# vitskvara/VBMatrixFactorization.jl

Measured on NVIDIA B200. Metric: VB iterations/s at 20000x200000x64 (dense vbmf, Float64), higher is better.
Workload: dtype f64

## Files before the change

vbmatrixfactorization.jl_b200/csrc/capi.cu:

```cuda
#include "../../include/vbmf_b200.h"
#include "common.cuh"
#include "gemm.cuh"
#include "kernels.cuh"

#include <atomic>
#include <type_traits>
#include <cstdarg>
#include <cstdlib>
#include <cstring>
#include <dlfcn.h>
#include <unistd.h>
#include <string>
#include <vector>
#include <algorithm>
#include <thread>

namespace vb {

static thread_local char g_err[1024] = "";
void set_error(const char* fmt, ...) {
    va_list ap;
    va_start(ap, fmt);
    vsnprintf(g_err, sizeof(g_err), fmt, ap);
    va_end(ap);
// ... 275 lines not shown
        if (comm_in != nullptr) c->comm = comm_in;
        else {
            if (nccl_id128 == nullptr) { set_error("world > 1 needs the NCCL unique id of rank 0"); delete c; return -1; }
            if (load_nccl()) { delete c; return -1; }
            NcclUniqueId id;
            memcpy(&id, nccl_id128, 128);
            int r = g_nccl.CommInitRank(&c->comm, c->world, id, rank);
            if (r != 0) { set_error("ncclCommInitRank failed: %s", g_nccl.GetErrorString ? g_nccl.GetErrorString(r) : "?"); delete c; return -1; }
        }
    }
    if (cudaMalloc(&c->d_tr, 64) != cudaSuccess) { set_error("cudaMalloc failed"); delete c; return -1; }
    *out = c;
    return 0;
}
extern "C" int vbmf_b200_ctx_create(int device, int rank, int world, const void* nccl_id128, void* cuda_stream,
                                    vbmf_b200_ctx** out) {
    return ctx_create_impl(device, rank, world, nccl_id128, nullptr, cuda_stream, out);
}
namespace vb {
int ctx_create_with_comm(int device, int rank, int world, void* comm, vbmf_b200_ctx** out) {
    return ctx_create_impl(device, rank, world, nullptr, comm, nullptr, out);
}
int nccl_comm_init_all(void** comms, int ndev, const int* devs) {
    if (load_nccl()) return -1;
    if (!g_nccl.CommInitAll) { set_error("the NCCL library has no ncclCommInitAll"); return -1; }
    VB_NCCL_OK(g_nccl.CommInitAll(comms, ndev, devs));
    return 0;
}
}

static void ctx_free_Z(vbmf_b200_ctx* c) {
    if (c->Z) cudaFree(c->Z);
    if (c->Zexp) cudaFree(c->Zexp);
    c->Z = nullptr; c->Zexp = nullptr; c->Z_bytes = 0;
    c->z_ready = false; c->z_failed = false;
}

static void ctx_free_Y(vbmf_b200_ctx* c) {
    ctx_free_Z(c);
    if (c->copy_st) cudaStreamSynchronize(c->copy_st);
    if (c->stat_st) cudaStreamSynchronize(c->stat_st);
    c->chunks_pending = 0; c->tr_pending = false;
    if (c->Y) cudaFree(c->Y);
    if (c->rowY2) cudaFree(c->rowY2);
    if (c->stats_part) cudaFree(c->stats_part);
    c->Y = nullptr; c->rowY2 = nullptr; c->stats_part = nullptr; c->have_Y = false;
    c->Y_cap = 0; c->L_cap = 0;
}

extern "C" int vbmf_b200_ctx_destroy(vbmf_b200_ctx* c) {
    if (!c) return 0;
    cudaSetDevice(c->device);
    cudaStreamSynchronize(c->st);
    ctx_free_Y(c);
    if (c->d_tr) cudaFree(c->d_tr);
    px_release(c);
    if (c->px.wait_ns) cudaFree(c->px.wait_ns);
    if (c->batch_dev) cudaFree(c->batch_dev);
    if (c->batch_host) cudaFreeHost(c->batch_host);
    for (auto e : c->ev_k1) cudaEventDestroy(e);
    for (auto e : c->ev_k2) cudaEventDestroy(e);
    for (auto e : c->ev_ar) cudaEventDestroy(e);
    for (auto& e : c->ev_seg) cudaEventDestroy(e.second);
    for (auto e : c->ev_chunk) cudaEventDestroy(e);
    if (c->ev_stats) cudaEventDestroy(c->ev_stats);
    if (c->copy_st) { cudaStreamSynchronize(c->copy_st); cudaStreamDestroy(c->copy_st); }
    if (c->stat_st) { cudaStreamSynchronize(c->stat_st); cudaStreamDestroy(c->stat_st); }
    if (c->comm) g_nccl.CommDestroy(c->comm);
    if (c->own_stream) cudaStreamDestroy(c->st);
    delete c;
    return 0;
}

extern "C" int vbmf_b200_ctx_sync(vbmf_b200_ctx* c) {
    VB_CUDA_OK(cudaSetDevice(c->device));
    if (c->copy_st) VB_CUDA_OK(cudaStreamSynchronize(c->copy_st));
    if (c->stat_st) VB_CUDA_OK(cudaStreamSynchronize(c->stat_st));
    VB_CUDA_OK(cudaStreamSynchronize(c->st));
    return 0;
}

static int ctx_alloc_Y(vbmf_b200_ctx* c, int64_t L, int64_t Mloc, int64_t Mglob, int64_t off) {
    if (L <= 0 || Mloc < 0 || Mglob < Mloc || off < 0 || off + Mloc > Mglob) { set_error("bad Y geometry L=%lld M_local=%lld M_global=%lld offset=%lld", (long long)L, (long long)Mloc, (long long)Mglob, (long long)off); return -1; }
    if (L > 0x7fffff00LL || Mglob > 0x7fffff00LL) { set_error("L and M must fit in 31 bits"); return -1; }
    VB_CUDA_OK(cudaSetDevice(c->device));
    VB_CUDA_OK(cudaStreamSynchronize(c->st));
    if (c->copy_st) VB_CUDA_OK(cudaStreamSynchronize(c->copy_st));
    if (c->stat_st) VB_CUDA_OK(cudaStreamSynchronize(c->stat_st));
    c->chunks_pending = 0; c->tr_pending = false;
    const int ld = (int)((L + 1) & ~1LL);
    const size_t bytes = std::max<size_t>((size_t)ld * (size_t)std::max<int64_t>(Mloc, 1) * 8, 16);
    const bool reuse = c->Y != nullptr && c->rowY2 != nullptr && c->stats_part != nullptr && bytes <= c->Y_cap &&
                       c->Y_cap <= 2 * bytes + (64u << 20) && L <= c->L_cap;
    if (!reuse) {
        ctx_free_Y(c);
        VB_CUDA_OK(cudaMalloc(&c->Y, bytes));
        c->Y_cap = bytes;
        VB_CUDA_OK(cudaMalloc(&c->rowY2, (size_t)L * 8));
        VB_CUDA_OK(cudaMalloc(&c->stats_part, (size_t)(MAX_PARTS / 2) * L * 8));
        c->L_cap = (int)L;
    }
    c->have_Y = false;
    c->z_ready = false; c->z_failed = false;
    c->L = (int)L; c->Mloc = (int)Mloc; c->Mglob = (int)Mglob; c->moff = (int)off;
    c->ldY = ld;
    if (c->ldY != L) VB_CUDA_OK(cudaMemsetAsync(c->Y, 0, bytes, c->st));
    return 0;
}

static int ctx_finish_Y(vbmf_b200_ctx* c) {
    if (c->Mloc > 0) {
        if (make_tmap_2d(&c->tmY1, c->Y, (uint64_t)c->L, (uint64_t)c->Mloc, (uint64_t)c->ldY * 8, 16, 128)) return -1;
        if (make_tmap_2d(&c->tmY2, c->Y, (uint64_t)c->L, (uint64_t)c->Mloc, (uint64_t)c->ldY * 8, 16, 16)) return -1;
    }
    Dev d;
    memset(&d, 0, sizeof(d));
    d.L = c->L; d.Mloc = c->Mloc; d.Y = c->Y; d.ldY = c->ldY; d.rowY2 = c->rowY2; d.part = c->stats_part;
    if (k_y_stats(c->st, d, c->d_tr)) return -1;
    if (c->world > 1) {
        if (ctx_allreduce(c, c->rowY2, (size_t)c->L)) return -1;
        if (k_total(c->st, c->rowY2, c->L, c->d_tr)) return -1;
    }
    VB_CUDA_OK(cudaMemcpyAsync(&c->trYTY, c->d_tr, 8, cudaMemcpyDeviceToHost, c->st));
    VB_CUDA_OK(cudaStreamSynchronize(c->st));
    c->have_Y = true;
    return 0;
}

static int ctx_wait_upload(vbmf_b200_ctx* c) {
    if (c->chunks_pending > 0) {
        VB_CUDA_OK(cudaStreamWaitEvent(c->st, c->ev_stats, 0));
        c->chunks_pending = 0;
    }
    return 0;
}
static int ctx_host_trYTY(vbmf_b200_ctx* c) {
    if (c->tr_pending) {
        VB_CUDA_OK(cudaEventSynchronize(c->ev_stats));
        VB_CUDA_OK(cudaMemcpy(&c->trYTY, c->d_tr, 8, cudaMemcpyDeviceToHost));
        c->tr_pending = false;
    }
    return 0;
}
static size_t align_up(size_t x, size_t a) { return (x + a - 1) / a * a; }

static bool ctx_int8_wanted(const vbmf_b200_ctx* c, int64_t H) {
    return !c->simt && !c->gemm_dmma && H >= 1 && H <= 64 && c->Y != nullptr && c->Mloc > 0;
}
static int ctx_slices(vbmf_b200_ctx* c, bool* ok) {
    *ok = false;
    if (c->z_failed || c->Y == nullptr || c->Mloc <= 0) return 0;
    if (c->z_ready) { *ok = true; return 0; }
    const int ldZ = i8_ld(c->L);
    const size_t bytes = (size_t)8 * c->Mloc * ldZ;
    if (c->Z == nullptr || c->Z_bytes != bytes || c->ldZ != ldZ) {
        ctx_free_Z(c);
        if (cudaMalloc(&c->Z, bytes) != cudaSuccess || cudaMalloc(&c->Zexp, ((size_t)c->L + c->Mloc) * 4) != cudaSuccess) {
            cudaGetLastError();
            ctx_free_Z(c);
            c->z_failed = true;
            return 0;
        }
        c->Z_bytes = bytes; c->ldZ = ldZ;
    }
    if (i8_build_Y(c->st, c->Y, c->ldY, c->L, c->Mloc, c->Z, ldZ, c->Zexp, c->Zexp + c->L)) return -1;
    const uint64_t s1 = (uint64_t)ldZ, s2 = (uint64_t)ldZ * c->Mloc;
    if (make_tmap_3d_i8(&c->tmZ1, c->Z, (uint64_t)c->L, (uint64_t)c->Mloc, 8, s1, s2, 32, 128, 8, false)) return -1;
    if (make_tmap_3d_i8(&c->tmZ2, c->Z, (uint64_t)c->L, (uint64_t)c->Mloc, 8, s1, s2, 128, 32, 8, true)) return -1;
    c->z_ready = true;
    *ok = true;
    return 0;
}
static void i8_plans(int L, int M, int H, int num_sms, int* S1, int* kbs1, int* S, int* kchunk) {
    plan_splitk_ytb(L, M, H, num_sms, S1, kbs1);
    *kbs1 = (*kbs1 + 1) & ~1;
    const int nkb = (L + 15) / 16;
    *S1 = std::max(1, (nkb + *kbs1 - 1) / *kbs1);
    plan_splitk(L, M, H, num_sms, S, kchunk);
    *kchunk = (*kchunk + 31) / 32 * 32;
    *S = std::max(1, (M + *kchunk - 1) / *kchunk);
}
struct I8Operands {
    char* mem = nullptr;
    uint8_t *Wb = nullptr, *Wa = nullptr;
    int *Gb = nullptr, *Ga = nullptr;
    int ldM = 0;
    CUtensorMap tmWb, tmWa;
    I8Operands() = default;
    I8Operands(const I8Operands&) = delete;
    I8Operands& operator=(const I8Operands&) = delete;
    ~I8Operands() { if (mem) cudaFree(mem); }
};
static int i8_operands_alloc(I8Operands* o, int L, int M, int H, int S, bool* ok) {
    *ok = false;
    const int Hp = i8_hpad(H), ldZ = i8_ld(L);
    o->ldM = i8_ld(std::max(M, 1));
    const size_t nb = align_up((size_t)8 * Hp * ldZ, 256), na = align_up((size_t)8 * Hp * o->ldM, 256);
    const size_t gb = align_up((size_t)Hp * 4, 256), ga = align_up((size_t)S * Hp * 4, 256);
    if (cudaMalloc(&o->mem, nb + na + gb + ga) != cudaSuccess) { cudaGetLastError(); o->mem = nullptr; return 0; }
    o->Wb = (uint8_t*)o->mem; o->Wa = o->Wb + nb; o->Gb = (int*)(o->Wa + na); o->Ga = (int*)((char*)o->Gb + gb);
    if (make_tmap_3d_i8(&o->tmWb, o->Wb, (uint64_t)L, (uint64_t)Hp, 8, (uint64_t)ldZ, (uint64_t)ldZ * Hp, 32, (uint32_t)Hp, 8, false)) return -1;
    if (M > 0 && make_tmap_3d_i8(&o->tmWa, o->Wa, (uint64_t)M, (uint64_t)Hp, 8, (uint64_t)o->ldM, (uint64_t)o->ldM * Hp, 32, (uint32_t)Hp, 8, false)) return -1;
    *ok = true;
    return 0;
}
static int i8_k1(vbmf_b200_ctx* c, I8Operands* o, const double* B, int ldB, int H, double* P, int S1, int kbs1, const Scalars* sc) {
    const int* F = c->Zexp;
    const int* E = c->Zexp + c->L;
    if (i8_slice_B(c->st, B, ldB, c->L, H, F, o->Wb, c->ldZ, o->Gb, sc)) return -1;
    return launch_gemm_i8(c->st, false, &c->tmZ1, &o->tmWb, P, c->Mloc, c->L, S1, kbs1 * 16, H, E, o->Gb, 0,
                          (size_t)c->Mloc * H, (size_t)H, 1, sc, c->num_sms);
}
static int i8_k2(vbmf_b200_ctx* c, I8Operands* o, const double* A, int H, double* Qpart, int ldQ, int S, int kchunk, const Scalars* sc) {
    const int* F = c->Zexp;
    const int* E = c->Zexp + c->L;
    if (i8_slice_A(c->st, A, c->Mloc, H, E, kchunk, S, o->Wa, o->ldM, o->Ga, sc)) return -1;
    return launch_gemm_i8(c->st, true, &c->tmZ2, &o->tmWa, Qpart, c->L, c->Mloc, S, kchunk, H, F, o->Ga, i8_hpad(H),
                          (size_t)H * ldQ, 1, (size_t)ldQ, sc, c->num_sms);
}

static int attach_Y_chunked(vbmf_b200_ctx* c, const double* Y, int64_t ldY, int64_t chunk_cols) {
    if (!c->copy_st) VB_CUDA_OK(cudaStreamCreateWithFlags(&c->copy_st, cudaStreamNonBlocking));
    if (!c->stat_st) VB_CUDA_OK(cudaStreamCreateWithFlags(&c->stat_st, cudaStreamNonBlocking));
    if (!c->ev_stats) VB_CUDA_OK(cudaEventCreateWithFlags(&c->ev_stats, cudaEventDisableTiming));
    c->chunk_c0.clear(); c->chunk_n.clear();
    for (int64_t c0 = 0; c0 < c->Mloc; c0 += chunk_cols) { c->chunk_c0.push_back((int)c0); c->chunk_n.push_back((int)std::min<int64_t>(chunk_cols, c->Mloc - c0)); }
    const size_t nch = c->chunk_c0.size();
    while (c->ev_chunk.size() < nch) { cudaEvent_t e; VB_CUDA_OK(cudaEventCreateWithFlags(&e, cudaEventDisableTiming)); c->ev_chunk.push_back(e); }
    cudaEvent_t e0;
    VB_CUDA_OK(cudaEventCreateWithFlags(&e0, cudaEventDisableTiming));
    VB_CUDA_OK(cudaEventRecord(e0, c->st));
    VB_CUDA_OK(cudaStreamWaitEvent(c->copy_st, e0, 0));
    VB_CUDA_OK(cudaStreamWaitEvent(c->stat_st, e0, 0));
    VB_CUDA_OK(cudaEventDestroy(e0));
    Dev d;
    memset(&d, 0, sizeof(d));
    d.L = c->L; d.Mloc = c->Mloc; d.Y = c->Y; d.ldY = c->ldY; d.rowY2 = c->rowY2; d.part = c->stats_part;
    for (size_t k = 0; k < nch; ++k) {
        const size_t c0 = (size_t)c->chunk_c0[k], n = (size_t)c->chunk_n[k];
        if (ldY == c->L && c->ldY == c->L)
            VB_CUDA_OK(cudaMemcpyAsync(c->Y + c0 * c->ldY, Y + c0 * (size_t)ldY, (size_t)c->L * n * 8, cudaMemcpyHostToDevice, c->copy_st));
        else
            VB_CUDA_OK(cudaMemcpy2DAsync(c->Y + c0 * c->ldY, (size_t)c->ldY * 8, Y + c0 * (size_t)ldY, (size_t)ldY * 8, (size_t)c->L * 8, n,
                                         cudaMemcpyHostToDevice, c->copy_st));
        VB_CUDA_OK(cudaEventRecord(c->ev_chunk[k], c->copy_st));
        VB_CUDA_OK(cudaStreamWaitEvent(c->stat_st, c->ev_chunk[k], 0));
        if (k_y_stats_chunk(c->stat_st, d, (int)c0, (int)n, k == 0 ? 1 : 0)) return -1;
    }
    if (c->world > 1) VB_NCCL_OK(g_nccl.AllReduce(c->rowY2, c->rowY2, (size_t)c->L, 8, 0, c->comm, c->stat_st));
    if (k_total(c->stat_st, c->rowY2, c->L, c->d_tr)) return -1;
    VB_CUDA_OK(cudaEventRecord(c->ev_stats, c->stat_st));
    if (make_tmap_2d(&c->tmY1, c->Y, (uint64_t)c->L, (uint64_t)c->Mloc, (uint64_t)c->ldY * 8, 16, 128)) return -1;
    if (make_tmap_2d(&c->tmY2, c->Y, (uint64_t)c->L, (uint64_t)c->Mloc, (uint64_t)c->ldY * 8, 16, 16)) return -1;
    c->chunks_pending = (int)nch;
    c->tr_pending = true;
    c->trYTY = nan("");
    c->have_Y = true;
    return 0;
}

extern "C" int vbmf_b200_attach_Y(vbmf_b200_ctx* c, const double* Y, int64_t L, int64_t M_local, int64_t ldY,
                                  int64_t M_global, int64_t col_offset) {
    if (!c || (!Y && M_local > 0)) { set_error("attach_Y: NULL argument"); return -1; }
    if (ldY < L) { set_error("attach_Y: ldY < L"); return -1; }
    if (ctx_alloc_Y(c, L, M_local, M_global, col_offset)) return -1;
    {
        const char* e = getenv("VBMF_B200_ATTACH_CHUNK_MB");
        const double chunk_mb = e ? atof(e) : 2048.0;
        const double col_bytes = (double)c->ldY * 8.0;
        int64_t chunk_cols = (int64_t)(chunk_mb * 1048576.0 / col_bytes) / 128 * 128;
        if (chunk_cols < 128) chunk_cols = 128;
        if (chunk_mb > 0 && M_local >= 2 * chunk_cols && !c->simt) return attach_Y_chunked(c, Y, ldY, chunk_cols);
    }
    if (M_local > 0) {
        if (ldY == L && c->ldY == L) {
            VB_CUDA_OK(cudaMemcpyAsync(c->Y, Y, (size_t)L * (size_t)M_local * 8, cudaMemcpyHostToDevice, c->st));
        } else {
            VB_CUDA_OK(cudaMemcpy2DAsync(c->Y, (size_t)c->ldY * 8, Y, (size_t)ldY * 8, (size_t)L * 8, (size_t)M_local,
                                         cudaMemcpyHostToDevice, c->st));
        }
    }
    return ctx_finish_Y(c);
}

extern "C" int vbmf_b200_set_shape(vbmf_b200_ctx* c, int64_t L, int64_t M_local, int64_t M_global, int64_t col_offset) {
    if (!c) { set_error("set_shape: NULL ctx"); return -1; }
    if (L <= 0 || M_local < 0 || M_global < M_local || col_offset < 0 || col_offset + M_local > M_global || L > 0x7fffff00LL || M_global > 0x7fffff00LL) {
        set_error("set_shape: bad geometry"); return -1;
    }
    VB_CUDA_OK(cudaSetDevice(c->device));
    VB_CUDA_OK(cudaStreamSynchronize(c->st));
    ctx_free_Y(c);
    c->L = (int)L; c->Mloc = (int)M_local; c->Mglob = (int)M_global; c->moff = (int)col_offset;
    c->ldY = (int)((L + 1) & ~1LL);
    c->trYTY = nan("");
    c->have_Y = true;
    return 0;
}

extern "C" int vbmf_b200_synth_Y(vbmf_b200_ctx* c, int64_t L, int64_t M_local, int64_t M_global, int64_t col_offset,
                                 int rank, double noise, uint64_t seed) {
    if (!c) { set_error("synth_Y: NULL ctx"); return -1; }
    if (ctx_alloc_Y(c, L, M_local, M_global, col_offset)) return -1;
    if (k_synth(c->st, c->Y, c->ldY, c->L, c->Mloc, c->moff, rank, noise, seed)) return -1;
    return ctx_finish_Y(c);
}

extern "C" int vbmf_b200_preprocess_Y(vbmf_b200_ctx* c, double lambda, int64_t* L_out, int64_t* used_rows) {
    if (!c || !c->have_Y || !c->Y) { set_error("preprocess_Y: no Y attached"); return -1; }
    VB_CUDA_OK(cudaSetDevice(c->device));
    if (ctx_wait_upload(c) || ctx_host_trYTY(c)) return -1;
    const int L = c->L, M = c->Mloc;
    cudaStream_t st = c->st;
    double *mu = nullptr, *den = nullptr, *rs = nullptr;
    VB_CUDA_OK(cudaMalloc(&mu, (size_t)L * 8));
    VB_CUDA_OK(cudaMalloc(&den, (size_t)L * 8));
    VB_CUDA_OK(cudaMalloc(&rs, (size_t)L * 8));
    int rc = 0;
    rc = k_row_pass(st, c->Y, c->ldY, L, M, 0, nullptr, nullptr, c->stats_part, mu);
    if (!rc) rc = ctx_allreduce(c, mu, (size_t)L);
    if (!rc) rc = k_finish_stats(st, mu, L, (double)c->Mglob, 0);
    if (!rc) rc = k_row_pass(st, c->Y, c->ldY, L, M, 1, mu, nullptr, c->stats_part, den);
    if (!rc) rc = ctx_allreduce(c, den, (size_t)L);
    if (!rc) rc = k_finish_stats(st, den, L, (double)c->Mglob, 1);
    if (!rc) rc = k_row_pass(st, c->Y, c->ldY, L, M, 2, mu, den, c->stats_part, rs);
    if (!rc) rc = ctx_allreduce(c, rs, (size_t)L);
    std::vector<double> hrs((size_t)L);
    if (!rc && cudaMemcpyAsync(hrs.data(), rs, (size_t)L * 8, cudaMemcpyDeviceToHost, st) != cudaSuccess) { set_error("preprocess_Y: copy failed"); rc = -1; }
    if (!rc && cudaStreamSynchronize(st) != cudaSuccess) { set_error("preprocess_Y: sync failed"); rc = -1; }
    cudaFree(mu); cudaFree(den); cudaFree(rs);
    if (rc) return rc;
    std::vector<int> rows;
    for (int l = 0; l < L; ++l) if (hrs[l] >= 1e-5) rows.push_back(l);
    const int Lnew = (int)rows.size();
    if (Lnew == 0) { set_error("preprocess_Y: every row is constant, nothing left"); return -1; }
    c->z_ready = false; c->z_failed = false;
    if (Lnew == L) {
        if (k_scale_all(st, c->Y, (size_t)c->ldY * (size_t)std::max(M, 1), lambda)) return -1;
    } else {
        const int ldn = (Lnew + 1) & ~1;
        double* Yn = nullptr;
        int* drows = nullptr;
        const size_t bytes = std::max<size_t>((size_t)ldn * (size_t)std::max(M, 1) * 8, 16);
        VB_CUDA_OK(cudaMalloc(&Yn, bytes));
        VB_CUDA_OK(cudaMalloc(&drows, (size_t)Lnew * 4));
        VB_CUDA_OK(cudaMemsetAsync(Yn, 0, bytes, st));
        VB_CUDA_OK(cudaMemcpyAsync(drows, rows.data(), (size_t)Lnew * 4, cudaMemcpyHostToDevice, st));
        if (k_compact_rows(st, c->Y, c->ldY, Yn, ldn, drows, Lnew, M, lambda)) return -1;
        VB_CUDA_OK(cudaStreamSynchronize(st));
        cudaFree(drows);
        cudaFree(c->Y);
        c->Y = Yn; c->Y_cap = bytes; c->L = Lnew; c->ldY = ldn;
    }
    if (L_out) *L_out = Lnew;
    if (used_rows) for (int k = 0; k < Lnew; ++k) used_rows[k] = rows[k] + 1;
// ... 1603 lines not shown
```

vbmatrixfactorization.jl_b200/csrc/gemm.cuh:

```cuda
#pragma once
#include "common.cuh"

namespace vb {

typedef CUresult (*PFN_encodeTiled)(CUtensorMap*, CUtensorMapDataType, cuuint32_t, void*, const cuuint64_t*,
                                    const cuuint64_t*, const cuuint32_t*, const cuuint32_t*, CUtensorMapInterleave,
                                    CUtensorMapSwizzle, CUtensorMapL2promotion, CUtensorMapFloatOOBfill);
PFN_encodeTiled tmap_encoder();

int make_tmap_2d(CUtensorMap* out, const void* base, uint64_t dim0, uint64_t dim1, uint64_t stride1_bytes,
                 uint32_t box0, uint32_t box1);

struct GemmGeometry {
    int bn;
    int ctas_per_sm;
    int stages;
};
GemmGeometry gemm_geometry(int H);
int gemm_init_device();

int launch_gemm_ytb(cudaStream_t st, const CUtensorMap* tmY, const CUtensorMap* tmB, double* P,
                    int M, int L, int H, int ldP, int S, int kb_per_split, size_t slab_stride, const Scalars* sc, int num_sms);
void plan_splitk_ytb(int L, int M, int H, int num_sms, int* S, int* kb_per_split);

int launch_gemm_ya(cudaStream_t st, const CUtensorMap* tmY, const CUtensorMap* tmA, double* Qpart,
                   int L, int M, int H, int ldQ, int kchunk, int S, const Scalars* sc, int num_sms);

int plan_streamk(int L, int M, int H, int num_sms, int* kq, int* nk, int* grid, int* smax);
int launch_gemm_ya_sk(cudaStream_t st, const CUtensorMap* tmY, const CUtensorMap* tmA, double* Qpart, double* Q, int L, int M, int H,
                      int ldQ, int kq, int nk, int grid, const Scalars* sc);
int launch_reduce_q_sk(cudaStream_t st, const double* Qpart, double* Q, int L, int M, int H, int ldQ, int nk, int grid, const Scalars* sc);

void plan_splitk(int L, int M, int H, int num_sms, int* S, int* kchunk);

inline int i8_hpad(int H) { return (H + 15) / 16 * 16; }
inline int i8_ld(int n) { return (n + 15) / 16 * 16; }
int gemm_i8_init_device();
int make_tmap_3d_i8(CUtensorMap* out, const void* base, uint64_t d0, uint64_t d1, uint64_t d2, uint64_t s1, uint64_t s2,
                    uint32_t b0, uint32_t b1, uint32_t b2, bool swizzle128);
int i8_build_Y(cudaStream_t st, const double* Y, int ldY, int L, int M, uint8_t* Z, int ldZ, int* F, int* E);
int i8_slice_B(cudaStream_t st, const double* B, int ldB, int L, int H, const int* F, uint8_t* W, int ldZ, int* G, const Scalars* sc);
int i8_slice_A(cudaStream_t st, const double* A, int M, int H, const int* E, int kchunk, int S, uint8_t* W, int ldM, int* G, const Scalars* sc);
int launch_gemm_i8(cudaStream_t st, bool mn, const CUtensorMap* tmA, const CUtensorMap* tmB, double* out, int nrows, int kdim,
                   int S, int klen, int H, const int* rowexp, const int* colexp, int cstride, size_t slab, size_t rs, size_t hs,
                   const Scalars* sc, int num_sms);

int launch_gemm_ytb_simt(cudaStream_t st, const double* Y, int ldY, const double* B, int ldB, double* P,
                         int M, int L, int H, int ldP, const Scalars* sc);
int launch_gemm_ya_simt(cudaStream_t st, const double* Y, int ldY, const double* A, double* Qpart,
                        int L, int M, int H, int ldQ, int kchunk, int S, const Scalars* sc);

}
```

vbmatrixfactorization.jl_b200/csrc/gemm_int8.cu:

```cuda
#include "gemm.cuh"
#include <algorithm>

namespace vb {
namespace i8k {

constexpr int TM = 128;
constexpr int KB = 32;
constexpr int NSL = 8;
constexpr int STAGES = 4;
constexpr int A_BYTES = NSL * TM * KB;
constexpr int B_BYTES = NSL * 64 * KB;
constexpr int SB = A_BYTES + B_BYTES;
constexpr int SMEM = STAGES * SB + 1024 + 256;
constexpr int SEG_KB = 16384 / KB;
constexpr int EXP_NONE = -(1 << 30);

__device__ __forceinline__ uint32_t smem_u32(const void* p) { return (uint32_t)__cvta_generic_to_shared(p); }
__device__ __forceinline__ void mbar_init(uint32_t bar, uint32_t count) {
    asm volatile("mbarrier.init.shared::cta.b64 [%0], %1;" ::"r"(bar), "r"(count) : "memory");
}
__device__ __forceinline__ void mbar_expect_tx(uint32_t bar, uint32_t bytes) {
    asm volatile("mbarrier.arrive.expect_tx.shared::cta.b64 _, [%0], %1;" ::"r"(bar), "r"(bytes) : "memory");
}
__device__ __forceinline__ void mbar_arrive(uint32_t bar) {
    asm volatile("mbarrier.arrive.shared::cta.b64 _, [%0];" ::"r"(bar) : "memory");
}
__device__ __forceinline__ void mbar_wait(uint32_t bar, uint32_t parity) {
    uint32_t ok;
    do {
        asm volatile(
            "{\n\t.reg .pred p;\n\t"
            "mbarrier.try_wait.parity.shared::cta.b64 p, [%1], %2;\n\t"
            "selp.u32 %0, 1, 0, p;\n\t}"
            : "=r"(ok) : "r"(bar), "r"(parity) : "memory");
    } while (!ok);
}
__device__ __forceinline__ void tma_load_3d(uint32_t dst, const CUtensorMap* tm, uint32_t bar, int c0, int c1, int c2) {
    asm volatile(
        "cp.async.bulk.tensor.3d.shared::cluster.global.mbarrier::complete_tx::bytes [%0], [%1, {%3, %4, %5}], [%2];"
        ::"r"(dst), "l"(tm), "r"(bar), "r"(c0), "r"(c1), "r"(c2) : "memory");
}
__device__ __forceinline__ void tc_fence_before() { asm volatile("tcgen05.fence::before_thread_sync;" ::: "memory"); }
__device__ __forceinline__ void tc_fence_after() { asm volatile("tcgen05.fence::after_thread_sync;" ::: "memory"); }
__device__ __forceinline__ void tc_commit(uint32_t bar) {
    asm volatile("tcgen05.commit.cta_group::1.mbarrier::arrive::one.shared::cluster.b64 [%0];" ::"r"(bar) : "memory");
}
__device__ __forceinline__ void mma_i8(uint32_t d, uint64_t a, uint64_t b, uint32_t idesc, uint32_t acc) {
    asm volatile(
        "{\n\t.reg .pred p;\n\tsetp.ne.b32 p, %4, 0;\n\t"
        "tcgen05.mma.cta_group::1.kind::i8 [%0], %1, %2, %3, p;\n\t}"
        ::"r"(d), "l"(a), "l"(b), "r"(idesc), "r"(acc) : "memory");
}
__device__ __forceinline__ void tmem_ld8(uint32_t taddr, uint32_t (&v)[8]) {
    asm volatile("tcgen05.ld.sync.aligned.32x32b.x8.b32 {%0,%1,%2,%3,%4,%5,%6,%7}, [%8];"
                 : "=r"(v[0]), "=r"(v[1]), "=r"(v[2]), "=r"(v[3]), "=r"(v[4]), "=r"(v[5]), "=r"(v[6]), "=r"(v[7])
                 : "r"(taddr) : "memory");
}
__device__ __forceinline__ void tmem_wait_ld() { asm volatile("tcgen05.wait::ld.sync.aligned;" ::: "memory"); }

__device__ __forceinline__ uint64_t sdesc(uint32_t addr, uint32_t lbo, uint32_t sbo, uint32_t layout) {
    return (uint64_t)((addr & 0x3FFFFu) >> 4) | ((uint64_t)(lbo >> 4) << 16) | ((uint64_t)(sbo >> 4) << 32) | (1ull << 46) |
           ((uint64_t)layout << 61);
}
constexpr uint32_t LAYOUT_SW128 = 2, LAYOUT_SW32 = 6;

__device__ __forceinline__ int exp_of(double x) {
    if (x == 0.0 || !isfinite(x)) return EXP_NONE;
    int e;
    frexp(x, &e);
    return e;
}
__device__ __forceinline__ int exp_fix(int e) { return e <= EXP_NONE ? 0 : e; }

__device__ __forceinline__ void slice4(const double (&w)[4], uint32_t (&out)[NSL]) {
#pragma unroll
    for (int i = 0; i < NSL; ++i) out[i] = 0u;
#pragma unroll
    for (int q = 0; q < 4; ++q) {
        double t = w[q];
#pragma unroll
        for (int i = 0; i < NSL; ++i) {
            t *= 128.0;
            const double s = trunc(t);
            t -= s;
            out[i] |= ((uint32_t)(int)s & 0xffu) << (8 * q);
        }
    }
}

__device__ __forceinline__ int block_max_int(int v, int* red) {
#pragma unroll
    for (int o = 16; o > 0; o >>= 1) v = max(v, __shfl_xor_sync(0xffffffffu, v, o));
    const int w = threadIdx.x >> 5, l = threadIdx.x & 31;
    __syncthreads();
    if (l == 0) red[w] = v;
    __syncthreads();
    if (w == 0) {
        v = l < (int)(blockDim.x >> 5) ? red[l] : EXP_NONE;
#pragma unroll
        for (int o = 16; o > 0; o >>= 1) v = max(v, __shfl_xor_sync(0xffffffffu, v, o));
        if (l == 0) red[0] = v;
    }
    __syncthreads();
    return red[0];
}

__global__ void __launch_bounds__(256) y_row_exp_kernel(const double* __restrict__ Y, int ldY, int L, int M, int* __restrict__ F) {
    const int l = blockIdx.x * blockDim.x + threadIdx.x;
    if (l >= L) return;
    int e = EXP_NONE;
    for (int m = blockIdx.y; m < M; m += gridDim.y) e = max(e, exp_of(Y[(size_t)m * ldY + l]));
    atomicMax(F + l, e);
}

__global__ void __launch_bounds__(256) y_slices_kernel(const double* __restrict__ Y, int ldY, int L, int M, const int* __restrict__ F,
                                                       int* __restrict__ E, uint8_t* __restrict__ Z, int ldZ) {
    __shared__ int red[32];
    const int m = blockIdx.x;
    const double* y = Y + (size_t)m * ldY;
    int e = EXP_NONE;
    for (int l = threadIdx.x; l < L; l += blockDim.x) {
        const int ey = exp_of(y[l]);
        if (ey > EXP_NONE) e = max(e, ey - exp_fix(F[l]));
    }
    const int Em = exp_fix(block_max_int(e, red));
    if (threadIdx.x == 0) E[m] = Em;
    const size_t plane = (size_t)M * ldZ;
    for (int l4 = threadIdx.x; l4 < ldZ / 4; l4 += blockDim.x) {
        double w[4];
#pragma unroll
        for (int q = 0; q < 4; ++q) {
            const int l = 4 * l4 + q;
            w[q] = l < L ? ldexp(y[l], -(exp_fix(F[l]) + Em)) : 0.0;
        }
        uint32_t s[NSL];
        slice4(w, s);
#pragma unroll
        for (int i = 0; i < NSL; ++i) reinterpret_cast<uint32_t*>(Z + i * plane + (size_t)m * ldZ)[l4] = s[i];
    }
}

__global__ void __launch_bounds__(512) b_slices_kernel(const double* __restrict__ B, int ldB, int L, int H, int Hp, const int* __restrict__ F,
                                                       uint8_t* __restrict__ W, int ldZ, int* __restrict__ G, const Scalars* __restrict__ sc) {
    if (sc != nullptr && !sc->active) return;
    __shared__ int red[32];
    const int h = blockIdx.x;
    const double* b = B + (size_t)h * ldB;
    int e = EXP_NONE;
    if (h < H)
        for (int l = threadIdx.x; l < L; l += blockDim.x) {
            const int eb = exp_of(b[l]);
            if (eb > EXP_NONE) e = max(e, eb + exp_fix(F[l]));
        }
    const int Gh = exp_fix(block_max_int(e, red));
    if (threadIdx.x == 0) G[h] = Gh;
    const size_t plane = (size_t)Hp * ldZ;
    for (int l4 = threadIdx.x; l4 < ldZ / 4; l4 += blockDim.x) {
        double w[4];
#pragma unroll
        for (int q = 0; q < 4; ++q) {
            const int l = 4 * l4 + q;
            w[q] = (h < H && l < L) ? ldexp(b[l], exp_fix(F[l]) - Gh) : 0.0;
        }
        uint32_t s[NSL];
        slice4(w, s);
#pragma unroll
        for (int i = 0; i < NSL; ++i) reinterpret_cast<uint32_t*>(W + i * plane + (size_t)h * ldZ)[l4] = s[i];
    }
}

__global__ void __launch_bounds__(256) a_exp_kernel(const double* __restrict__ A, int M, int H, int Hp, const int* __restrict__ E, int kchunk,
                                                    int* __restrict__ G, const Scalars* __restrict__ sc) {
    if (sc != nullptr && !sc->active) return;
    const int h = threadIdx.x & 63;
    if (h >= H) return;
    const int m0 = blockIdx.x * 256, m1 = min(M, m0 + 256);
    int cur = -1, e = EXP_NONE;
    for (int m = m0 + (threadIdx.x >> 6); m < m1; m += 4) {
        const int c = m / kchunk;
        if (c != cur) {
            if (cur >= 0 && e > EXP_NONE) atomicMax(G + cur * Hp + h, e);
            cur = c; e = EXP_NONE;
        }
        const int ea = exp_of(A[(size_t)m * H + h]);
        if (ea > EXP_NONE) e = max(e, ea + E[m]);
    }
    if (cur >= 0 && e > EXP_NONE) atomicMax(G + cur * Hp + h, e);
}

__global__ void __launch_bounds__(256) a_slices_kernel(const double* __restrict__ A, int M, int H, int Hp, const int* __restrict__ E, int kchunk,
                                                       const int* __restrict__ G, uint8_t* __restrict__ W, int ldM, const Scalars* __restrict__ sc) {
    if (sc != nullptr && !sc->active) return;
    __shared__ double tile[64 * 64];
    const int m0 = blockIdx.x * 64;
    const int nm = min(64, M - m0);
    for (int t = threadIdx.x; t < nm * H; t += blockDim.x) tile[t] = A[(size_t)m0 * H + t];
    __syncthreads();
    const size_t plane = (size_t)Hp * ldM;
    for (int t = threadIdx.x; t < Hp * 16; t += blockDim.x) {
        const int h = t >> 4, g = t & 15;
        if (m0 + 4 * g >= ldM) continue;
        double w[4];
#pragma unroll
        for (int q = 0; q < 4; ++q) {
            const int r = 4 * g + q, m = m0 + r;
            w[q] = 0.0;
            if (h < H && r < nm) w[q] = ldexp(tile[r * H + h], E[m] - exp_fix(G[(m / kchunk) * Hp + h]));
        }
        uint32_t s[NSL];
        slice4(w, s);
#pragma unroll
        for (int i = 0; i < NSL; ++i) reinterpret_cast<uint32_t*>(W + i * plane + (size_t)h * ldM + m0)[g] = s[i];
    }
}

template <bool MN>
__global__ void __launch_bounds__(192, 1)
gemm_i8_kernel(const __grid_constant__ CUtensorMap tmA, const __grid_constant__ CUtensorMap tmB, double* __restrict__ out,
               int nrows, int kdim, int S, int klen, int H, int Hp, const int* __restrict__ rowexp,
               const int* __restrict__ colexp, int cstride, size_t slab, size_t rs, size_t hs, const Scalars* __restrict__ sc) {
    if (sc != nullptr && !sc->active) return;
    extern __shared__ uint8_t smem_raw[];
    const uint32_t base = (smem_u32(smem_raw) + 1023u) & ~1023u;
    const uint32_t full0 = base + STAGES * SB, empty0 = full0 + STAGES * 8;
    const uint32_t tfull = empty0 + STAGES * 8, tempty = tfull + 8, tslot = tempty + 8;
    uint32_t* tslot_ptr = reinterpret_cast<uint32_t*>(smem_raw + (tslot - smem_u32(smem_raw)));

    const int warp = threadIdx.x >> 5, lane = threadIdx.x & 31;
    const uint32_t ncols = Hp * NSL <= 128 ? 128 : (Hp * NSL <= 256 ? 256 : 512);
    if (threadIdx.x == 0) {
        for (int s = 0; s < STAGES; ++s) { mbar_init(full0 + 8 * s, 1); mbar_init(empty0 + 8 * s, 1); }
        mbar_init(tfull, 1);
        mbar_init(tempty, 4);
        asm volatile("fence.mbarrier_init.release.cluster;" ::: "memory");
        asm volatile("fence.proxy.async.shared::cta;" ::: "memory");
    }
    if (warp == 5) {
        asm volatile("tcgen05.alloc.cta_group::1.sync.aligned.shared::cta.b32 [%0], %1;" ::"r"(tslot), "r"(ncols) : "memory");
        asm volatile("tcgen05.relinquish_alloc_permit.cta_group::1.sync.aligned;" ::: "memory");
    }
    tc_fence_before();
    __syncthreads();
    tc_fence_after();
    const uint32_t tmem = *reinterpret_cast<volatile uint32_t*>(tslot_ptr);

    const int ntile = (nrows + TM - 1) / TM;
    const int nwork = ntile * S;
    const uint32_t tx_bytes = A_BYTES + NSL * Hp * KB;

    if (warp == 4) {
        if (lane == 0) {
            uint32_t it = 0;
            for (int w = blockIdx.x; w < nwork; w += gridDim.x) {
                const int r0 = (w % ntile) * TM, k0 = (w / ntile) * klen, k1 = min(kdim, k0 + klen);
                for (int k = k0; k < k1; k += KB, ++it) {
                    const uint32_t s = it % STAGES, ph = (it / STAGES) & 1;
                    mbar_wait(empty0 + 8 * s, ph ^ 1);
                    mbar_expect_tx(full0 + 8 * s, tx_bytes);
                    if (MN) tma_load_3d(base + s * SB, &tmA, full0 + 8 * s, r0, k, 0);
                    else tma_load_3d(base + s * SB, &tmA, full0 + 8 * s, k, r0, 0);
                    tma_load_3d(base + s * SB + A_BYTES, &tmB, full0 + 8 * s, k, 0, 0);
                }
            }
        }
    } else if (warp == 5) {
        if (lane == 0) {
            const uint32_t idesc0 = (2u << 4) | (1u << 7) | (1u << 10) | ((MN ? 1u : 0u) << 15) | ((uint32_t)(TM >> 4) << 24);
            uint32_t it = 0, sg = 0;
            for (int w = blockIdx.x; w < nwork; w += gridDim.x) {
                const int k0 = (w / ntile) * klen, k1 = min(kdim, k0 + klen);
                const int nkb = (k1 - k0 + KB - 1) / KB;
                for (int kb0 = 0; kb0 < nkb; kb0 += SEG_KB, ++sg) {
                    const int kb1 = min(nkb, kb0 + SEG_KB);
                    mbar_wait(tempty, (sg & 1) ^ 1);
                    tc_fence_after();
                    for (int kb = kb0; kb < kb1; ++kb, ++it) {
                        const uint32_t s = it % STAGES, ph = (it / STAGES) & 1;
                        mbar_wait(full0 + 8 * s, ph);
                        tc_fence_after();
                        const uint32_t a0 = base + s * SB, b0 = a0 + A_BYTES;
#pragma unroll
                        for (int i = 0; i < NSL; ++i) {
                            const uint64_t ad = MN ? sdesc(a0 + i * (TM * KB), 16, 1024, LAYOUT_SW128)
                                                   : sdesc(a0 + i * (TM * KB), 16, 256, LAYOUT_SW32);
                            const int ntot = Hp * (NSL - i);
                            for (int p = 0; p < ntot; p += 256) {
                                const int n = min(256, ntot - p);
                                const uint64_t bd = sdesc(b0 + p * KB, 16, 256, LAYOUT_SW32);
                                mma_i8(tmem + Hp * i + p, ad, bd, idesc0 | ((uint32_t)(n >> 3) << 17), (kb > kb0 || i > 0) ? 1u : 0u);
                            }
                        }
                        tc_commit(empty0 + 8 * s);
                    }
                    tc_commit(tfull);
                }
            }
        }
    } else {
        const uint32_t lane_base = (uint32_t)(warp * 32) << 16;
        uint32_t sg = 0;
        for (int w = blockIdx.x; w < nwork; w += gridDim.x) {
            const int tile = w % ntile, sp = w / ntile;
            const int k0 = sp * klen, k1 = min(kdim, k0 + klen);
            const int nkb = (k1 - k0 + KB - 1) / KB;
            const int row = tile * TM + warp * 32 + lane;
            const bool live = row < nrows;
            const int re = live ? rowexp[row] : 0;
            double* o = out + (size_t)sp * slab + (size_t)(live ? row : 0) * rs;
            const int* ce = colexp + (size_t)sp * cstride;
            for (int kb0 = 0; kb0 < nkb; kb0 += SEG_KB, ++sg) {
                mbar_wait(tfull, sg & 1);
                tc_fence_after();
                for (int h0 = 0; h0 < Hp; h0 += 8) {
                    uint32_t v[NSL][8];
#pragma unroll
                    for (int k = 0; k < NSL; ++k) tmem_ld8(tmem + lane_base + Hp * k + h0, v[k]);
                    tmem_wait_ld();
#pragma unroll
                    for (int c = 0; c < 8; ++c) {
                        const int h = h0 + c;
                        double acc = (double)(int)v[NSL - 1][c];
#pragma unroll
                        for (int k = NSL - 2; k >= 0; --k) acc = fma(acc, 0x1p-7, (double)(int)v[k][c]);
                        if (live && h < H) {
                            const double x = ldexp(acc, re + ce[h] - 14);
                            double* p = o + (size_t)h * hs;
                            *p = kb0 == 0 ? x : *p + x;
                        }
                    }
                }
                tc_fence_before();
                __syncwarp();
                if (lane == 0) mbar_arrive(tempty);
            }
        }
    }
    tc_fence_before();
    __syncthreads();
    if (warp == 5) {
        tc_fence_after();
        asm volatile("tcgen05.dealloc.cta_group::1.sync.aligned.b32 %0, %1;" ::"r"(tmem), "r"(ncols) : "memory");
    }
}

}
using namespace i8k;

int make_tmap_3d_i8(CUtensorMap* out, const void* base, uint64_t d0, uint64_t d1, uint64_t d2, uint64_t s1, uint64_t s2,
                    uint32_t b0, uint32_t b1, uint32_t b2, bool swizzle128) {
    PFN_encodeTiled enc = tmap_encoder();
    if (!enc) return -1;
    if ((reinterpret_cast<uintptr_t>(base) & 15) != 0 || (s1 & 15) != 0 || (s2 & 15) != 0) {
        set_error("INT8 tensor map needs a 16-byte aligned base and pitches (base=%p pitches %llu, %llu)", base,
                  (unsigned long long)s1, (unsigned long long)s2);
        return -1;
    }
    cuuint64_t dims[3] = {d0, d1, d2};
    cuuint64_t strides[2] = {s1, s2};
    cuuint32_t box[3] = {b0, b1, b2};
    cuuint32_t estr[3] = {1, 1, 1};
    CUresult r = enc(out, CU_TENSOR_MAP_DATA_TYPE_UINT8, 3, const_cast<void*>(base), dims, strides, box, estr,
                     CU_TENSOR_MAP_INTERLEAVE_NONE, swizzle128 ? CU_TENSOR_MAP_SWIZZLE_128B : CU_TENSOR_MAP_SWIZZLE_32B,
                     CU_TENSOR_MAP_L2_PROMOTION_L2_128B, CU_TENSOR_MAP_FLOAT_OOB_FILL_NONE);
    if (r != CUDA_SUCCESS) {
        set_error("cuTensorMapEncodeTiled (int8) failed with CUresult %d (dims %llu x %llu x %llu, box %u x %u x %u)", (int)r,
                  (unsigned long long)d0, (unsigned long long)d1, (unsigned long long)d2, b0, b1, b2);
        return -1;
    }
    return 0;
}

int gemm_i8_init_device() {
    VB_CUDA_OK(cudaFuncSetAttribute(gemm_i8_kernel<false>, cudaFuncAttributeMaxDynamicSharedMemorySize, SMEM));
    VB_CUDA_OK(cudaFuncSetAttribute(gemm_i8_kernel<true>, cudaFuncAttributeMaxDynamicSharedMemorySize, SMEM));
    return 0;
}

int i8_build_Y(cudaStream_t st, const double* Y, int ldY, int L, int M, uint8_t* Z, int ldZ, int* F, int* E) {
    if (L <= 0 || M <= 0) return 0;
    VB_CUDA_OK(cudaMemsetAsync(F, 0x80, (size_t)L * 4, st));
    dim3 g1((L + 255) / 256, std::min(M, 512));
    y_row_exp_kernel<<<g1, 256, 0, st>>>(Y, ldY, L, M, F);
    VB_LAUNCH_OK();
    y_slices_kernel<<<M, 256, 0, st>>>(Y, ldY, L, M, F, E, Z, ldZ);
    VB_LAUNCH_OK();
    return 0;
}

int i8_slice_B(cudaStream_t st, const double* B, int ldB, int L, int H, const int* F, uint8_t* W, int ldZ, int* G, const Scalars* sc) {
    const int Hp = i8_hpad(H);
    b_slices_kernel<<<Hp, 512, 0, st>>>(B, ldB, L, H, Hp, F, W, ldZ, G, sc);
    VB_LAUNCH_OK();
    return 0;
}

int i8_slice_A(cudaStream_t st, const double* A, int M, int H, const int* E, int kchunk, int S, uint8_t* W, int ldM, int* G, const Scalars* sc) {
    if (M <= 0) return 0;
    const int Hp = i8_hpad(H);
    VB_CUDA_OK(cudaMemsetAsync(G, 0x80, (size_t)S * Hp * 4, st));
    a_exp_kernel<<<(M + 255) / 256, 256, 0, st>>>(A, M, H, Hp, E, kchunk, G, sc);
    VB_LAUNCH_OK();
    a_slices_kernel<<<(ldM + 63) / 64, 256, 0, st>>>(A, M, H, Hp, E, kchunk, G, W, ldM, sc);
    VB_LAUNCH_OK();
    return 0;
}

int launch_gemm_i8(cudaStream_t st, bool mn, const CUtensorMap* tmA, const CUtensorMap* tmB, double* out, int nrows, int kdim,
                   int S, int klen, int H, const int* rowexp, const int* colexp, int cstride, size_t slab, size_t rs, size_t hs,
                   const Scalars* sc, int num_sms) {
    if (H > 64) { set_error("H = %d > 64 is not supported by the INT8 contraction", H); return -1; }
    if (klen % KB != 0) { set_error("INT8 split-K chunk %d is not a multiple of %d", klen, KB); return -1; }
    if (nrows <= 0 || kdim <= 0 || H <= 0) return 0;
    const int nwork = ((nrows + TM - 1) / TM) * S;
    const int grid = std::max(1, std::min(nwork, num_sms));
    if (mn) gemm_i8_kernel<true><<<grid, 192, SMEM, st>>>(*tmA, *tmB, out, nrows, kdim, S, klen, H, i8_hpad(H), rowexp, colexp, cstride, slab, rs, hs, sc);
    else gemm_i8_kernel<false><<<grid, 192, SMEM, st>>>(*tmA, *tmB, out, nrows, kdim, S, klen, H, i8_hpad(H), rowexp, colexp, cstride, slab, rs, hs, sc);
    VB_LAUNCH_OK();
    return 0;
}

}
```

Measured before the change: 53.14.

## Use signed base-256 digit slicing with seven int8 planes instead of eight base-128

Replaces the base-128 truncation slicing of FP64 operands into eight int8 planes with a signed base-256 digit decomposition of a 55-bit fixed-point integer, needing only seven planes. This cuts the bytes of Y slices, the staged shared memory per pipeline stage, and the number of int8 MMAs and TMEM reads in the emulated DGEMM by about one eighth. Exponent selection is adjusted to leave headroom for rounding into the top digit. The risk is INT32 accumulator overflow between flushes and changed rounding of the emulated FP64 result.

```diff
diff --git a/vbmatrixfactorization.jl_b200/csrc/capi.cu b/vbmatrixfactorization.jl_b200/csrc/capi.cu
--- a/vbmatrixfactorization.jl_b200/csrc/capi.cu
+++ b/vbmatrixfactorization.jl_b200/csrc/capi.cu
@@ -451,7 +451,7 @@
     if (c->z_failed || c->Y == nullptr || c->Mloc <= 0) return 0;
     if (c->z_ready) { *ok = true; return 0; }
     const int ldZ = i8_ld(c->L);
-    const size_t bytes = (size_t)8 * c->Mloc * ldZ;
+    const size_t bytes = (size_t)I8_NSL * c->Mloc * ldZ;
     if (c->Z == nullptr || c->Z_bytes != bytes || c->ldZ != ldZ) {
         ctx_free_Z(c);
         if (cudaMalloc(&c->Z, bytes) != cudaSuccess || cudaMalloc(&c->Zexp, ((size_t)c->L + c->Mloc) * 4) != cudaSuccess) {
@@ -464,8 +464,8 @@
     }
     if (i8_build_Y(c->st, c->Y, c->ldY, c->L, c->Mloc, c->Z, ldZ, c->Zexp, c->Zexp + c->L)) return -1;
     const uint64_t s1 = (uint64_t)ldZ, s2 = (uint64_t)ldZ * c->Mloc;
-    if (make_tmap_3d_i8(&c->tmZ1, c->Z, (uint64_t)c->L, (uint64_t)c->Mloc, 8, s1, s2, 32, 128, 8, false)) return -1;
-    if (make_tmap_3d_i8(&c->tmZ2, c->Z, (uint64_t)c->L, (uint64_t)c->Mloc, 8, s1, s2, 128, 32, 8, true)) return -1;
+    if (make_tmap_3d_i8(&c->tmZ1, c->Z, (uint64_t)c->L, (uint64_t)c->Mloc, I8_NSL, s1, s2, 32, 128, I8_NSL, false)) return -1;
+    if (make_tmap_3d_i8(&c->tmZ2, c->Z, (uint64_t)c->L, (uint64_t)c->Mloc, I8_NSL, s1, s2, 128, 32, I8_NSL, true)) return -1;
     c->z_ready = true;
     *ok = true;
     return 0;
@@ -494,12 +494,12 @@
     *ok = false;
     const int Hp = i8_hpad(H), ldZ = i8_ld(L);
     o->ldM = i8_ld(std::max(M, 1));
-    const size_t nb = align_up((size_t)8 * Hp * ldZ, 256), na = align_up((size_t)8 * Hp * o->ldM, 256);
+    const size_t nb = align_up((size_t)I8_NSL * Hp * ldZ, 256), na = align_up((size_t)I8_NSL * Hp * o->ldM, 256);
     const size_t gb = align_up((size_t)Hp * 4, 256), ga = align_up((size_t)S * Hp * 4, 256);
     if (cudaMalloc(&o->mem, nb + na + gb + ga) != cudaSuccess) { cudaGetLastError(); o->mem = nullptr; return 0; }
     o->Wb = (uint8_t*)o->mem; o->Wa = o->Wb + nb; o->Gb = (int*)(o->Wa + na); o->Ga = (int*)((char*)o->Gb + gb);
-    if (make_tmap_3d_i8(&o->tmWb, o->Wb, (uint64_t)L, (uint64_t)Hp, 8, (uint64_t)ldZ, (uint64_t)ldZ * Hp, 32, (uint32_t)Hp, 8, false)) return -1;
-    if (M > 0 && make_tmap_3d_i8(&o->tmWa, o->Wa, (uint64_t)M, (uint64_t)Hp, 8, (uint64_t)o->ldM, (uint64_t)o->ldM * Hp, 32, (uint32_t)Hp, 8, false)) return -1;
+    if (make_tmap_3d_i8(&o->tmWb, o->Wb, (uint64_t)L, (uint64_t)Hp, I8_NSL, (uint64_t)ldZ, (uint64_t)ldZ * Hp, 32, (uint32_t)Hp, I8_NSL, false)) return -1;
+    if (M > 0 && make_tmap_3d_i8(&o->tmWa, o->Wa, (uint64_t)M, (uint64_t)Hp, I8_NSL, (uint64_t)o->ldM, (uint64_t)o->ldM * Hp, 32, (uint32_t)Hp, I8_NSL, false)) return -1;
     *ok = true;
     return 0;
 }
diff --git a/vbmatrixfactorization.jl_b200/csrc/gemm.cuh b/vbmatrixfactorization.jl_b200/csrc/gemm.cuh
--- a/vbmatrixfactorization.jl_b200/csrc/gemm.cuh
+++ b/vbmatrixfactorization.jl_b200/csrc/gemm.cuh
@@ -33,6 +33,7 @@
 
 void plan_splitk(int L, int M, int H, int num_sms, int* S, int* kchunk);
 
+constexpr int I8_NSL = 7;
 inline int i8_hpad(int H) { return (H + 15) / 16 * 16; }
 inline int i8_ld(int n) { return (n + 15) / 16 * 16; }
 int gemm_i8_init_device();
diff --git a/vbmatrixfactorization.jl_b200/csrc/gemm_int8.cu b/vbmatrixfactorization.jl_b200/csrc/gemm_int8.cu
--- a/vbmatrixfactorization.jl_b200/csrc/gemm_int8.cu
+++ b/vbmatrixfactorization.jl_b200/csrc/gemm_int8.cu
@@ -6,13 +6,16 @@
 
 constexpr int TM = 128;
 constexpr int KB = 32;
-constexpr int NSL = 8;
+constexpr int NSL = I8_NSL;
 constexpr int STAGES = 4;
 constexpr int A_BYTES = NSL * TM * KB;
 constexpr int B_BYTES = NSL * 64 * KB;
 constexpr int SB = A_BYTES + B_BYTES;
+static_assert(SB % 1024 == 0 && A_BYTES % 1024 == 0, "stage layout must stay 1024-byte aligned");
 constexpr int SMEM = STAGES * SB + 1024 + 256;
+static_assert(SMEM <= 227 * 1024, "stage ring exceeds the shared memory of one CTA");
 constexpr int SEG_KB = 16384 / KB;
+static_assert((long long)SEG_KB * KB * NSL * 128 * 128 < (1ll << 31), "level 6 may overflow INT32 between flushes");
 constexpr int EXP_NONE = -(1 << 30);
 
 __device__ __forceinline__ uint32_t smem_u32(const void* p) { return (uint32_t)__cvta_generic_to_shared(p); }
@@ -70,20 +73,27 @@
     frexp(x, &e);
     return e;
 }
+__device__ __forceinline__ int exp_digits(double x) {
+    if (x == 0.0 || !isfinite(x)) return EXP_NONE;
+    int e;
+    const double m = frexp(x, &e);
+    return fabs(m) > 127.0 / 128.0 ? e + 1 : e;
+}
 __device__ __forceinline__ int exp_fix(int e) { return e <= EXP_NONE ? 0 : e; }
 
-__device__ __forceinline__ void slice4(const double (&w)[4], uint32_t (&out)[NSL]) {
+__device__ __forceinline__ long long fixed55(double x, int e) { return __double2ll_rn(ldexp(x, 55 - e)); }
+
+__device__ __forceinline__ void digits4(const long long (&x)[4], uint32_t (&out)[NSL]) {
 #pragma unroll
     for (int i = 0; i < NSL; ++i) out[i] = 0u;
 #pragma unroll
     for (int q = 0; q < 4; ++q) {
-        double t = w[q];
-#pragma unroll
-        for (int i = 0; i < NSL; ++i) {
-            t *= 128.0;
-            const double s = trunc(t);
-            t -= s;
-            out[i] |= ((uint32_t)(int)s & 0xffu) << (8 * q);
+        long long t = x[q];
+#pragma unroll
+        for (int i = NSL - 1; i >= 0; --i) {
+            const int d = (int8_t)(t & 255);
+            out[i] |= ((uint32_t)t & 0xffu) << (8 * q);
+            t = (t - d) >> 8;
         }
     }
 }
@@ -120,21 +130,21 @@
     const double* y = Y + (size_t)m * ldY;
     int e = EXP_NONE;
     for (int l = threadIdx.x; l < L; l += blockDim.x) {
-        const int ey = exp_of(y[l]);
+        const int ey = exp_digits(y[l]);
         if (ey > EXP_NONE) e = max(e, ey - exp_fix(F[l]));
     }
     const int Em = exp_fix(block_max_int(e, red));
     if (threadIdx.x == 0) E[m] = Em;
     const size_t plane = (size_t)M * ldZ;
     for (int l4 = threadIdx.x; l4 < ldZ / 4; l4 += blockDim.x) {
-        double w[4];
+        long long x[4];
 #pragma unroll
         for (int q = 0; q < 4; ++q) {
             const int l = 4 * l4 + q;
-            w[q] = l < L ? ldexp(y[l], -(exp_fix(F[l]) + Em)) : 0.0;
+            x[q] = l < L ? fixed55(y[l], exp_fix(F[l]) + Em) : 0;
         }
         uint32_t s[NSL];
-        slice4(w, s);
+        digits4(x, s);
 #pragma unroll
         for (int i = 0; i < NSL; ++i) reinterpret_cast<uint32_t*>(Z + i * plane + (size_t)m * ldZ)[l4] = s[i];
     }
@@ -149,21 +159,21 @@
     int e = EXP_NONE;
     if (h < H)
         for (int l = threadIdx.x; l < L; l += blockDim.x) {
-            const int eb = exp_of(b[l]);
+            const int eb = exp_digits(b[l]);
             if (eb > EXP_NONE) e = max(e, eb + exp_fix(F[l]));
         }
     const int Gh = exp_fix(block_max_int(e, red));
     if (threadIdx.x == 0) G[h] = Gh;
     const size_t plane = (size_t)Hp * ldZ;
     for (int l4 = threadIdx.x; l4 < ldZ / 4; l4 += blockDim.x) {
-        double w[4];
+        long long x[4];
 #pragma unroll
         for (int q = 0; q < 4; ++q) {
             const int l = 4 * l4 + q;
-            w[q] = (h < H && l < L) ? ldexp(b[l], exp_fix(F[l]) - Gh) : 0.0;
+            x[q] = (h < H && l < L) ? fixed55(b[l], Gh - exp_fix(F[l])) : 0;
         }
         uint32_t s[NSL];
-        slice4(w, s);
+        digits4(x, s);
 #pragma unroll
         for (int i = 0; i < NSL; ++i) reinterpret_cast<uint32_t*>(W + i * plane + (size_t)h * ldZ)[l4] = s[i];
     }
@@ -182,7 +192,7 @@
             if (cur >= 0 && e > EXP_NONE) atomicMax(G + cur * Hp + h, e);
             cur = c; e = EXP_NONE;
         }
-        const int ea = exp_of(A[(size_t)m * H + h]);
+        const int ea = exp_digits(A[(size_t)m * H + h]);
         if (ea > EXP_NONE) e = max(e, ea + E[m]);
     }
     if (cur >= 0 && e > EXP_NONE) atomicMax(G + cur * Hp + h, e);
@@ -200,15 +210,15 @@
     for (int t = threadIdx.x; t < Hp * 16; t += blockDim.x) {
         const int h = t >> 4, g = t & 15;
         if (m0 + 4 * g >= ldM) continue;
-        double w[4];
+        long long x[4];
 #pragma unroll
         for (int q = 0; q < 4; ++q) {
             const int r = 4 * g + q, m = m0 + r;
-            w[q] = 0.0;
-            if (h < H && r < nm) w[q] = ldexp(tile[r * H + h], E[m] - exp_fix(G[(m / kchunk) * Hp + h]));
+            x[q] = 0;
+            if (h < H && r < nm) x[q] = fixed55(tile[r * H + h], exp_fix(G[(m / kchunk) * Hp + h]) - E[m]);
         }
         uint32_t s[NSL];
-        slice4(w, s);
+        digits4(x, s);
 #pragma unroll
         for (int i = 0; i < NSL; ++i) reinterpret_cast<uint32_t*>(W + i * plane + (size_t)h * ldM + m0)[g] = s[i];
     }
@@ -321,7 +331,7 @@
                         const int h = h0 + c;
                         double acc = (double)(int)v[NSL - 1][c];
 #pragma unroll
-                        for (int k = NSL - 2; k >= 0; --k) acc = fma(acc, 0x1p-7, (double)(int)v[k][c]);
+                        for (int k = NSL - 2; k >= 0; --k) acc = fma(acc, 0x1p-8, (double)(int)v[k][c]);
                         if (live && h < H) {
                             const double x = ldexp(acc, re + ce[h] - 14);
                             double* p = o + (size_t)h * hs;
```

New measurement: 63.44, median of 6. +19.4%, better.
